# Spockuto/drand

Measured on AMD Instinct MI355X. Metric: beacons verified/s (batch chain verify), higher is better.
Workload: dtype u32 (381-bit Montgomery, 12x32-bit limbs); 1 GPU; configs[1]: 1000000-round chained beacon history per GPU, chain.VerifyBeacon per round; beacons_per_gpu=1000000, segment_len=64, parallelism=range-shard x1

## Files before the change

drand_amd/csrc/blsverify.cpp:

```cpp
#include <hip/hip_runtime.h>
#include <sys/random.h>

#include <algorithm>
#include <initializer_list>
#include <cerrno>
#include <cstdarg>
#include <cstdio>
#include <cstring>
#include <string>
#include <cstdlib>
#include <thread>
#include <vector>

#include "../../include/blsverify.h"
#include "../../include/blsverify_testing.h"
#include "kernels.h"
#include "engine_ctx.h"
#include "testops_list.h"

void release_workspace(blsv_ctx* c) {
  for (DBuf* d : {&c->H, &c->HQ, &c->S, &c->F, &c->FW, &c->LN, &c->h_inf, &c->s_inf, &c->cls}) d->release();
  c->cap = 0;
}

// ... 266 lines not shown
int blsv_test_lagrange(const uint32_t* idx, size_t t, uint32_t* out) {
  if (!idx || !out) return BLSV_EINVAL;
  for (size_t i = 0; i < t; i++)
    for (size_t j = 0; j < i; j++)
      if (idx[i] == idx[j]) return BLSV_EINVAL;
  host_lagrange(idx, t, out);
  return BLSV_OK;
}

struct PkSel {
  const uint32_t* tab;
  const uint8_t* inf;
  const uint32_t* idx;
};

static bool serial_stages() {
  static const bool on = [] {
    const char* e = getenv("BLSV_SERIAL_STAGES");
    return e && e[0] == '1';
  }();
  return on;
}

template <typename HashFn>
static int run_head(blsv_ctx* c, const uint8_t* d_sigs, size_t stride, size_t offset, size_t base, size_t cnt,
                    hipStream_t st, HashFn hash) {
  if (serial_stages()) {
    {
      StageTimer tm(c, ST_DECOMP, cnt, st);
      blsk::launch_decompress_g2(d_sigs, stride, offset, base, cnt, c->S.as<uint32_t>(), c->s_inf.as<uint8_t>(),
                                 c->cls.as<uint8_t>(), st);
    }
    StageTimer tm(c, ST_HASH, cnt, st);
    hash();
    return BLSV_OK;
  }
  HIPCHK(c, hipEventRecord(c->fork_ev, st));
  HIPCHK(c, hipStreamWaitEvent(c->side, c->fork_ev, 0));
  {
    StageTimer tm(c, ST_DECOMP, cnt, c->side);
    blsk::launch_decompress_g2(d_sigs, stride, offset, base, cnt, c->S.as<uint32_t>(), c->s_inf.as<uint8_t>(),
                               c->cls.as<uint8_t>(), c->side);
  }
  HIPCHK(c, hipEventRecord(c->join_ev, c->side));
  {
    StageTimer tm(c, ST_HASH, cnt, st);
    hash();
  }
  HIPCHK(c, hipStreamWaitEvent(st, c->join_ev, 0));
  return BLSV_OK;
}

static int run_tail(blsv_ctx* c, const uint8_t* d_sigs, size_t stride, size_t offset, size_t base, size_t cnt,
                    const PkSel& pk, uint64_t* d_bitmap, unsigned long long* d_first_bad, uint8_t* d_cls_out,
                    hipStream_t st, uint64_t label0 = 0) {
  (void)d_sigs;
  (void)stride;
  (void)offset;
  {
    StageTimer tm(c, ST_MILLER, cnt, st);
    blsk::launch_miller(pk.tab, pk.inf, pk.idx, c->H.as<uint32_t>(), c->h_inf.as<uint8_t>(), c->S.as<uint32_t>(),
                        c->s_inf.as<uint8_t>(), c->cls.as<uint8_t>(), cnt, c->F.as<uint32_t>(), c->LN.as<uint32_t>(),
                        std::min(cnt, kLineSub), c->FW.as<uint32_t>(), st);
  }
  {
    StageTimer tm(c, ST_FEXP, cnt, st);
    blsk::launch_final_exp(c->F.as<uint32_t>(), c->FW.as<uint32_t>(), cnt, c->cls.as<uint8_t>(), st,
                           c->LN.as<uint32_t>());
  }
  {
    StageTimer tm(c, ST_FINISH, cnt, st);
    blsk::launch_finish(c->cls.as<uint8_t>(), base, cnt, d_bitmap, d_first_bad, label0, st);
  }
  if (d_cls_out) HIPCHK(c, hipMemcpyAsync(d_cls_out + base, c->cls.p, cnt, hipMemcpyDeviceToDevice, st));
  HIPCHK(c, hipGetLastError());
  return BLSV_OK;
}

static void bitmap_words_to_bytes(const std::vector<uint64_t>& w, size_t n, uint8_t* out) {
  for (size_t i = 0; i < (n + 7) / 8; i++) {
    uint8_t b = (uint8_t)(w[i / 8] >> (8 * (i % 8)));
    if (i == (n + 7) / 8 - 1 && (n % 8)) b &= (uint8_t)((1u << (n % 8)) - 1);
    out[i] = b;
  }
}

// ... 33 lines not shown
    uint8_t* cls = reject_class;
    if (!cls) {
      own.resize(n);
      cls = own.data();
    }
    HIPCHK(c, download_sync(c, {{cls, c->cls.p, n}}));
    uint64_t fb = UINT64_MAX;
    for (size_t i = 0; i < n; i++) {
      if (cls[i] != BLSV_REJ_OK && fb == UINT64_MAX) fb = i;
      if (ok_bitmap) {
        if (i % 8 == 0) ok_bitmap[i / 8] = 0;
        ok_bitmap[i / 8] |= (uint8_t)((cls[i] == BLSV_REJ_OK) << (i % 8));
      }
    }
    if (first_bad_idx) *first_bad_idx = fb;
    return BLSV_OK;
  }
  HIPCHK(c, c->bitmap.ensure(words * 8 + 8));
  HIPCHK(c, c->first_bad.ensure(8));
  HIPCHK(c, hipMemsetAsync(c->first_bad.p, 0xff, 8, c->stream));
  if (reject_class) HIPCHK(c, c->misc.ensure(n + 64));
  for (size_t base = 0; base < n; base += c->cap) {
    const size_t cnt = std::min(c->cap, n - base);
    rc = run_head(c, d_sigs, stride, offset, base, cnt, c->stream, [&]() { hash(base, cnt); });
    if (rc) return rc;
    rc = run_tail(c, d_sigs, stride, offset, base, cnt, pk, c->bitmap.as<uint64_t>(),
                  c->first_bad.as<unsigned long long>(), reject_class ? c->misc.as<uint8_t>() : nullptr, c->stream);
    if (rc) return rc;
  }
  std::vector<uint64_t> w(words + 1, 0);
  uint64_t fb = UINT64_MAX;
  HIPCHK(c, download_sync(c, {{w.data(), c->bitmap.p, words * 8},
                              {&fb, c->first_bad.p, 8},
                              {reject_class, c->misc.p, reject_class ? n : 0}}));
  if (ok_bitmap) bitmap_words_to_bytes(w, n, ok_bitmap);
  if (first_bad_idx) *first_bad_idx = fb;
  return BLSV_OK;
}

static PkSel group_pk(blsv_ctx* c) { return {c->commits.as<uint32_t>(), c->commit_inf.as<uint8_t>(), nullptr}; }

static bool use_rlc(const blsv_ctx* c, size_t n) { return n > c->lat_max && n >= 2 * c->rlc.group; }

static int rlc_draw_seed(blsv_ctx* c, uint32_t (&w)[8]) {
  uint8_t s[32];
  if (c->rlc.seed_pinned) {
    memcpy(s, c->rlc.seed, 32);
// ... 15 lines not shown

static int rlc_sums(blsv_ctx* c, size_t base, size_t cnt, const uint32_t (&seed)[8], hipStream_t st) {
  rlc_state& r = c->rlc;
  const size_t ng = blsk::rlc_groups(cnt, r.group), cap = round64(ng);
  HIPCHK(c, r.part.ensure(2 * blsk::kRlcPartWords * blsk::rlc_lanes(cnt) * 4));
  HIPCHK(c, r.gH.ensure(cap * blsk::H_WORDS * 4));
  HIPCHK(c, r.gS.ensure(cap * blsk::S_WORDS * 4));
  HIPCHK(c, r.g_hinf.ensure(cap));
  HIPCHK(c, r.g_sinf.ensure(cap));
  HIPCHK(c, r.gcls.ensure(cap));
  StageTimer tm(c, ST_RLC, cnt, st);
  blsk::launch_rlc_sums(c->H.as<uint32_t>(), c->h_inf.as<uint8_t>(), c->S.as<uint32_t>(), c->s_inf.as<uint8_t>(),
                        c->cls.as<uint8_t>(), cnt, base, seed, r.group, r.part.as<uint32_t>(), r.gH.as<uint32_t>(),
                        r.g_hinf.as<uint8_t>(), r.gS.as<uint32_t>(), r.g_sinf.as<uint8_t>(), st);
  return BLSV_OK;
}

static void rlc_pairing_check(blsv_ctx* c, const uint32_t* H, const uint8_t* h_inf, const uint32_t* S,
                              const uint8_t* s_inf, uint8_t* cls, size_t cnt, hipStream_t st) {
  const PkSel pk = group_pk(c);
  {
    StageTimer tm(c, ST_MILLER, cnt, st);
    blsk::launch_miller(pk.tab, pk.inf, pk.idx, H, h_inf, S, s_inf, cls, cnt, c->F.as<uint32_t>(),
                        c->LN.as<uint32_t>(), std::min(cnt, kLineSub), c->FW.as<uint32_t>(), st);
  }
  StageTimer tm(c, ST_FEXP, cnt, st);
  blsk::launch_final_exp(c->F.as<uint32_t>(), c->FW.as<uint32_t>(), cnt, cls, st, c->LN.as<uint32_t>());
}

static int run_tail_rlc(blsv_ctx* c, size_t base, size_t cnt, const uint32_t (&seed)[8], uint64_t* d_bitmap,
                        unsigned long long* d_first_bad, uint8_t* d_cls_out, hipStream_t st, uint64_t label0 = 0) {
  rlc_state& r = c->rlc;
  const size_t G = r.group, ng = blsk::rlc_groups(cnt, G);
  int rc = rlc_sums(c, base, cnt, seed, st);
  if (rc) return rc;
  HIPCHK(c, hipMemsetAsync(r.gcls.p, 0, ng, st));
  rlc_pairing_check(c, r.gH.as<uint32_t>(), r.g_hinf.as<uint8_t>(), r.gS.as<uint32_t>(), r.g_sinf.as<uint8_t>(),
                    r.gcls.as<uint8_t>(), ng, st);
  HIPCHK(c, hipGetLastError());
  HIPCHK(c, r.host.ensure(kMaxChunk / kRlcGroupMin * 5 + 16));
  uint8_t* verdict = r.host.as<uint8_t>();
  HIPCHK(c, hipMemcpyAsync(verdict, r.gcls.p, ng, hipMemcpyDeviceToHost, st));
  HIPCHK(c, hipStreamSynchronize(st));
  uint32_t* fail_list = reinterpret_cast<uint32_t*>(verdict + ((ng + 7) & ~size_t(7)));
  size_t nf = 0;
  for (size_t g = 0; g < ng; g++)
    if (verdict[g] != BLSV_REJ_OK) fail_list[nf++] = (uint32_t)g;
// ... 25 lines not shown
    StageTimer tm(c, ST_FINISH, cnt, st);
    blsk::launch_finish(c->cls.as<uint8_t>(), base, cnt, d_bitmap, d_first_bad, label0, st);
  }
  if (d_cls_out) HIPCHK(c, hipMemcpyAsync(d_cls_out + base, c->cls.p, cnt, hipMemcpyDeviceToDevice, st));
  HIPCHK(c, hipGetLastError());
  return BLSV_OK;
}

template <typename HashFn>
static int verify_driver_rlc(blsv_ctx* c, size_t n, const uint8_t* d_sigs, HashFn hash, uint8_t* ok_bitmap,
                             uint64_t* first_bad_idx, uint8_t* reject_class) {
  const size_t words = (n + 63) / 64;
  int rc = ensure_workspace(c, n);
  if (rc) return rc;
  uint32_t seed[8];
  rc = rlc_draw_seed(c, seed);
  if (rc) return rc;
  HIPCHK(c, c->bitmap.ensure(words * 8 + 8));
  HIPCHK(c, c->first_bad.ensure(8));
  HIPCHK(c, hipMemsetAsync(c->first_bad.p, 0xff, 8, c->stream));
  if (reject_class) HIPCHK(c, c->misc.ensure(n + 64));
  for (size_t base = 0; base < n; base += c->cap) {
    const size_t cnt = std::min(c->cap, n - base);
    rc = run_head(c, d_sigs, 96, 0, base, cnt, c->stream, [&]() { hash(base, cnt); });
    if (rc) return rc;
    rc = run_tail_rlc(c, base, cnt, seed, c->bitmap.as<uint64_t>(), c->first_bad.as<unsigned long long>(),
                      reject_class ? c->misc.as<uint8_t>() : nullptr, c->stream);
    if (rc) return rc;
  }
  std::vector<uint64_t> w(words + 1, 0);
  uint64_t fb = UINT64_MAX;
  HIPCHK(c, download_sync(c, {{w.data(), c->bitmap.p, words * 8},
                              {&fb, c->first_bad.p, 8},
                              {reject_class, c->misc.p, reject_class ? n : 0}}));
  if (ok_bitmap) bitmap_words_to_bytes(w, n, ok_bitmap);
  if (first_bad_idx) *first_bad_idx = fb;
  return BLSV_OK;
}

static int decode_g1(blsv_ctx* c, const uint8_t* pk48, size_t cnt, DBuf& tab, DBuf& inf, std::vector<uint8_t>& cls) {
  HIPCHK(c, tab.ensure(cnt * blsk::G1_WORDS * 4));
  HIPCHK(c, inf.ensure(cnt));
  HIPCHK(c, c->g1_cls.ensure(cnt));
  HIPCHK(c, c->misc.ensure(cnt * 48));
  HIPCHK(c, hipMemcpyAsync(c->misc.p, pk48, cnt * 48, hipMemcpyHostToDevice, c->stream));
  blsk::launch_decompress_g1(c->misc.as<uint8_t>(), cnt, tab.as<uint32_t>(), inf.as<uint8_t>(),
                             c->g1_cls.as<uint8_t>(), c->stream);
// ... 38 lines not shown
  memcpy(h + o_idx, idx, n * 4);
  memcpy(h + o_sig, sigs96, n * 96);
  if (mbytes) memcpy(h + o_msg, msgs, mbytes);
  HIPCHK(c, c->arena.ensure(total));
  HIPCHK(c, c->misc.ensure(n + 64));
  HIPCHK(c, hipMemcpyAsync(c->arena.p, h, total, hipMemcpyHostToDevice, c->stream));
  uint8_t* d = c->arena.as<uint8_t>();
  const uint64_t* d_off = reinterpret_cast<const uint64_t*>(d);
  const uint32_t* d_len = reinterpret_cast<const uint32_t*>(d + o_len);
  const uint32_t* d_idx = reinterpret_cast<const uint32_t*>(d + o_idx);
  const uint8_t* d_sig = d + o_sig;
  const uint8_t* d_msg = d + o_msg;
  if (use_lat(c, n)) {
    blsk::launch_lat_messages(d_msg, d_off, d_len, d_sig, 96, 0, n, d_tab, d_tab_inf, d_idx, c->misc.as<uint8_t>(),
                              nullptr, nullptr, c->stream);
  } else {
    const size_t words = (n + 63) / 64;
    HIPCHK(c, c->bitmap.ensure(words * 8 + 8));
    HIPCHK(c, c->first_bad.ensure(8));
    HIPCHK(c, hipMemsetAsync(c->first_bad.p, 0xff, 8, c->stream));
    for (size_t base = 0; base < n; base += c->cap) {
      const size_t cnt = std::min(c->cap, n - base);
      const PkSel pk{d_tab, d_tab_inf, d_idx + base};
      rc = run_head(c, d_sig, 96, 0, base, cnt, c->stream, [&]() {
        blsk::launch_hash_messages(d_msg, d_off + base, d_len + base, cnt, c->H.as<uint32_t>(), c->h_inf.as<uint8_t>(),
                                   c->HQ.as<uint32_t>(), c->stream);
      });
      if (rc) return rc;
      rc = run_tail(c, d_sig, 96, 0, base, cnt, pk, c->bitmap.as<uint64_t>(), c->first_bad.as<unsigned long long>(),
                    c->misc.as<uint8_t>(), c->stream);
      if (rc) return rc;
    }
  }
  HIPCHK(c, hipGetLastError());
  HIPCHK(c, hipMemcpyAsync(h, c->misc.p, n, hipMemcpyDeviceToHost, c->stream));
  HIPCHK(c, hipStreamSynchronize(c->stream));
  memcpy(cls_out, h, n);
  return BLSV_OK;
}

extern "C" {

const char* blsv_version(void) { return "drand_amd blsverify 0.1 (gfx950)"; }

int blsv_device_count(void) {
  int n = 0;
  return hipGetDeviceCount(&n) == hipSuccess ? n : 0;
// ... 335 lines not shown
    HIPCHK(c, c->pp_inf.ensure(k));
    HIPCHK(c, c->sel.ensure(k * 4));
    ident.resize(k);
    for (size_t i = 0; i < k; i++) ident[i] = (uint32_t)i;
    HIPCHK(c, h2d(c, c->sel.p, ident.data(), k * 4));
    blsk::launch_pubpoly_eval(c->commits.as<uint32_t>(), c->commit_inf.as<uint8_t>(), (uint32_t)c->t,
                              c->idx.as<uint32_t>(), k, c->pp_tab.as<uint32_t>(), c->pp_inf.as<uint8_t>(), c->stream);
    pk = {c->pp_tab.as<uint32_t>(), c->pp_inf.as<uint8_t>(), c->sel.as<uint32_t>()};
  }
  HIPCHK(c, c->in_sigs.ensure(k * partial_len + 96));
  HIPCHK(c, h2d(c, c->in_sigs.p, partials, k * partial_len));
  if (use_lat(c, k)) {
    StageTimer tm(c, ST_LAT, k, c->stream);
    blsk::launch_lat_messages(c->in_msgs.as<uint8_t>(), c->in_off.as<uint64_t>(), c->in_len.as<uint32_t>(),
                              c->in_sigs.as<uint8_t>(), partial_len, 2, k, pk.tab, pk.inf, pk.idx, c->cls.as<uint8_t>(),
                              c->S.as<uint32_t>(), c->s_inf.as<uint8_t>(), c->stream);
    HIPCHK(c, hipGetLastError());
  } else {
    HIPCHK(c, c->bitmap.ensure(((k + 63) / 64) * 8 + 8));
    HIPCHK(c, c->first_bad.ensure(8));
    HIPCHK(c, hipMemsetAsync(c->first_bad.p, 0xff, 8, c->stream));
    blsk::launch_hash_messages(c->in_msgs.as<uint8_t>(), c->in_off.as<uint64_t>(), c->in_len.as<uint32_t>(), k,
                               c->H.as<uint32_t>(), c->h_inf.as<uint8_t>(), c->HQ.as<uint32_t>(), c->stream);
    rc = run_head(c, c->in_sigs.as<uint8_t>(), partial_len, 2, 0, k, c->stream, []() {});
    if (rc) return rc;
    rc = run_tail(c, c->in_sigs.as<uint8_t>(), partial_len, 2, 0, k, pk, c->bitmap.as<uint64_t>(),
                  c->first_bad.as<unsigned long long>(), nullptr, c->stream);
    if (rc) return rc;
  }
  HIPCHK(c, download_sync(c, {{cls.data(), c->cls.p, k}}));
  return BLSV_OK;
}

int blsv_verify_partials(blsv_ctx* c, const uint8_t* msg, size_t msg_len, const uint8_t* partials, size_t partial_len,
                         size_t k, uint8_t* ok, uint8_t* reject_class) {
  if (!c) return BLSV_EINVAL;
  if ((k && (!partials || !ok)) || (msg_len && !msg)) return fail(c, BLSV_EINVAL, "verify_partials: null arguments");
  (void)hipSetDevice(c->device);
  std::vector<uint8_t> cls;
  std::vector<uint32_t> index;
  int rc = partials_stage(c, msg, msg_len, partials, partial_len, k, cls, index);
  if (rc) return rc;
  for (size_t i = 0; i < k; i++) {
    ok[i] = cls[i] == BLSV_REJ_OK;
    if (reject_class) reject_class[i] = cls[i];
  }
  return BLSV_OK;
// ... 350 lines not shown
                            const uint8_t* d_seeds96, size_t seed0_len, const uint8_t* d_sigs96, size_t n,
                            uint64_t* d_bitmap, uint64_t* d_first_bad, uint8_t* d_reject_class, void* stream) {
  if (!c) return BLSV_EINVAL;
  if (!c->has_group) return fail(c, BLSV_ENOGROUP, "verify_chained_dev: no group key set");
  if (n && (!d_seeds96 || !d_sigs96 || !d_bitmap || !d_first_bad || (seed0_len != 32 && seed0_len != 96)))
    return fail(c, BLSV_EINVAL, "verify_chained_dev: bad arguments");
  if (seg_phase && (!seg_len || seg_phase >= seg_len))
    return fail(c, BLSV_EINVAL, "verify_chained_dev: seg_phase must be < seg_len");
  (void)hipSetDevice(c->device);
  hipStream_t st = stream ? (hipStream_t)stream : c->stream;
  HIPCHK(c, hipMemsetAsync(d_first_bad, 0xff, 8, st));
  int rc = ensure_workspace(c, n);
  if (rc) return rc;
  blsk::ChainedSrc src{d_sigs96, d_seeds96, first_round, seg_len ? seg_len : std::max<uint64_t>(n, 1),
                       (uint32_t)seed0_len, seg_phase};
  if (use_lat(c, n)) {
    const PkSel pk = group_pk(c);
    return run_lat(
        c, n, [&](uint8_t* cls) { blsk::launch_lat_chained(src, 0, n, pk.tab, pk.inf, cls, st); }, d_bitmap,
        (unsigned long long*)d_first_bad, d_reject_class, st, first_round);
  }
  for (size_t base = 0; base < n; base += c->cap) {
    const size_t cnt = std::min(c->cap, n - base);
    rc = run_head(c, d_sigs96, 96, 0, base, cnt, st, [&]() {
      blsk::launch_hash_chained(src, base, cnt, c->H.as<uint32_t>(), c->h_inf.as<uint8_t>(), c->HQ.as<uint32_t>(), st);
    });
    if (rc) return rc;
    rc = run_tail(c, d_sigs96, 96, 0, base, cnt, group_pk(c), d_bitmap, (unsigned long long*)d_first_bad,
                  d_reject_class, st, first_round);
    if (rc) return rc;
  }
  return BLSV_OK;
}

int blsv_generate_chained_dev(blsv_ctx* c, const uint8_t* sk32, uint64_t first_round, uint64_t seg_len,
                              const uint8_t* d_seeds96, size_t seed0_len, uint8_t* d_sigs96, size_t n, void* stream) {
  if (!c) return BLSV_EINVAL;
  if (!sk32 || (n && (!d_seeds96 || !d_sigs96)) || (seed0_len != 32 && seed0_len != 96))
    return fail(c, BLSV_EINVAL, "generate_chained_dev: bad arguments");
  (void)hipSetDevice(c->device);
  hipStream_t st = stream ? (hipStream_t)stream : c->stream;
  uint32_t sk[8];
  scalar_mod_r(sk32, sk);
  HIPCHK(c, c->sk.ensure(32));
  HIPCHK(c, hipMemcpyAsync(c->sk.p, sk, 32, hipMemcpyHostToDevice, st));
  blsk::ChainedSrc src{d_sigs96, d_seeds96, first_round, seg_len ? seg_len : std::max<uint64_t>(n, 1),
                       (uint32_t)seed0_len};
// ... 63 lines not shown
int blsv_verify_chained_rlc_dev(blsv_ctx* c, uint64_t first_round, uint64_t seg_len, uint64_t seg_phase,
                                const uint8_t* d_seeds96, size_t seed0_len, const uint8_t* d_sigs96, size_t n,
                                uint64_t* d_bitmap, uint64_t* d_first_bad, uint8_t* d_reject_class, void* stream) {
  if (!c) return BLSV_EINVAL;
  if (!use_rlc(c, n))
    return blsv_verify_chained_dev(c, first_round, seg_len, seg_phase, d_seeds96, seed0_len, d_sigs96, n, d_bitmap,
                                   d_first_bad, d_reject_class, stream);
  if (!c->has_group) return fail(c, BLSV_ENOGROUP, "verify_chained_rlc_dev: no group key set");
  if (!d_seeds96 || !d_sigs96 || !d_bitmap || !d_first_bad || (seed0_len != 32 && seed0_len != 96))
    return fail(c, BLSV_EINVAL, "verify_chained_rlc_dev: bad arguments");
  if (seg_phase && (!seg_len || seg_phase >= seg_len))
    return fail(c, BLSV_EINVAL, "verify_chained_rlc_dev: seg_phase must be < seg_len");
  (void)hipSetDevice(c->device);
  hipStream_t st = stream ? (hipStream_t)stream : c->stream;
  uint32_t seed[8];
  int rc = rlc_draw_seed(c, seed);
  if (rc) return rc;
  HIPCHK(c, hipMemsetAsync(d_first_bad, 0xff, 8, st));
  rc = ensure_workspace(c, n);
  if (rc) return rc;
  blsk::ChainedSrc src{d_sigs96, d_seeds96, first_round, seg_len ? seg_len : n, (uint32_t)seed0_len, seg_phase};
  for (size_t base = 0; base < n; base += c->cap) {
    const size_t cnt = std::min(c->cap, n - base);
    rc = run_head(c, d_sigs96, 96, 0, base, cnt, st, [&]() {
      blsk::launch_hash_chained(src, base, cnt, c->H.as<uint32_t>(), c->h_inf.as<uint8_t>(), c->HQ.as<uint32_t>(), st);
    });
    if (rc) return rc;
    rc = run_tail_rlc(c, base, cnt, seed, d_bitmap, (unsigned long long*)d_first_bad, d_reject_class, st, first_round);
    if (rc) return rc;
  }
  return BLSV_OK;
}

size_t blsv_set_rlc_group(blsv_ctx* c, size_t g) {
  if (!c) return 0;
  const size_t prev = c->rlc.group;
  size_t v = kRlcGroupMin;
  while (v * 2 <= g && v < kRlcGroupMax) v *= 2;
  c->rlc.group = v;
  return prev;
}

int blsv_rlc_stats(blsv_ctx* c, uint64_t* groups, uint64_t* groups_failed, uint64_t* items_exact) {
  if (!c) return BLSV_EINVAL;
  if (groups) *groups = c->rlc.groups;
  if (groups_failed) *groups_failed = c->rlc.groups_failed;
  if (items_exact) *items_exact = c->rlc.items_exact;
// ... 7 lines not shown
  return BLSV_OK;
}

int blsv_test_rlc_sums(blsv_ctx* c, uint64_t first_round, const uint8_t* prev0, size_t prev0_len,
                       const uint8_t* sigs96, size_t n, uint8_t* out_a96, uint8_t* out_b96) {
  if (!c) return BLSV_EINVAL;
  if (!n || !sigs96 || !prev0 || !out_a96 || !out_b96 || (prev0_len != 32 && prev0_len != 96))
    return fail(c, BLSV_EINVAL, "test_rlc_sums: bad arguments");
  (void)hipSetDevice(c->device);
  uint32_t seed[8];
  int rc = rlc_draw_seed(c, seed);
  if (rc) return rc;
  rc = ensure_workspace(c, n);
  if (rc) return rc;
  HIPCHK(c, c->in_sigs.ensure(n * 96 + 96));
  HIPCHK(c, c->seeds.ensure(96));
  HIPCHK(c, h2d(c, c->in_sigs.p, sigs96, n * 96));
  HIPCHK(c, h2d(c, c->seeds.p, prev0, prev0_len));
  blsk::ChainedSrc src{c->in_sigs.as<uint8_t>(), c->seeds.as<uint8_t>(), first_round, n, (uint32_t)prev0_len};
  rlc_state& r = c->rlc;
  size_t done = 0;
  for (size_t base = 0; base < n; base += c->cap) {
    const size_t cnt = std::min(c->cap, n - base), ng = blsk::rlc_groups(cnt, r.group);
    rc = run_head(c, c->in_sigs.as<uint8_t>(), 96, 0, base, cnt, c->stream, [&]() {
      blsk::launch_hash_chained(src, base, cnt, c->H.as<uint32_t>(), c->h_inf.as<uint8_t>(), c->HQ.as<uint32_t>(),
                                c->stream);
    });
    if (rc) return rc;
    rc = rlc_sums(c, base, cnt, seed, c->stream);
    if (rc) return rc;
    HIPCHK(c, r.out96.ensure(2 * ng * 96));
    uint8_t* d_out = r.out96.as<uint8_t>();
    blsk::launch_rlc_compress(r.gH.as<uint32_t>(), r.g_hinf.as<uint8_t>(), ng, d_out, c->stream);
    blsk::launch_rlc_compress(r.gS.as<uint32_t>(), r.g_sinf.as<uint8_t>(), ng, d_out + ng * 96, c->stream);
    HIPCHK(c, hipGetLastError());
    HIPCHK(c, hipMemcpyAsync(out_a96 + done * 96, d_out, ng * 96, hipMemcpyDeviceToHost, c->stream));
    HIPCHK(c, hipMemcpyAsync(out_b96 + done * 96, d_out + ng * 96, ng * 96, hipMemcpyDeviceToHost, c->stream));
    HIPCHK(c, hipStreamSynchronize(c->stream));
    c->io_up_off = 0;
    done += ng;
  }
  return (int)done;
}


static int tlock_prepare_sig(blsv_ctx* c, const uint8_t* sig96, hipStream_t st, uint8_t* sig_class) {
  tlock_state& t = c->tlock;
// ... 342 lines not shown
```

drand_amd/csrc/k_decomp.hip:

```cpp
#define BLS_FP2_KARA_INL 1
#include "kcommon.h"

namespace blsk {

#ifndef BLS_WPE_SUBGROUP
#define BLS_WPE_SUBGROUP 2
#endif

BLS_KERNEL(BLS_WPE_DECOMP) k_decompress_g2(const uint8_t* sigs, size_t stride, size_t offset, size_t base,
                                           size_t cnt, uint32_t* S, uint8_t* s_inf, uint8_t* cls) {
  size_t i = (size_t)blockIdx.x * TPB + threadIdx.x;
  if (i >= cnt) return;
  uint8_t buf[96];
  const uint8_t* p = sigs + (base + i) * stride + offset;
  for (int k = 0; k < 96; k++) buf[k] = p[k];
  g2a a;
  bool inf;
  uint8_t c = g2_decompress(buf, a, inf, false);
  if (c != REJ_OK) {
    a.x = fp2_zero();
    a.y = fp2_zero();
    inf = true;
  }
  st_fp2(S, cnt, i, 0, a.x);
// ... 63 lines not shown
  const bool in = i < cnt;
  const bool ok = in && cls[i] == REJ_OK;
  const bool bad = in && !ok;
  const unsigned long long okm = __ballot(ok);
  const unsigned long long badm = __ballot(bad);
  const int lane = threadIdx.x & 63;
  const size_t wave0 = i - lane;
  if (lane == 0 && wave0 < cnt) {
    bitmap[(base + wave0) >> 6] = okm;
    if (badm) atomicMin(first_bad, (unsigned long long)(label0 + base + wave0 + __builtin_ctzll(badm)));
  }
}

void launch_decompress_g2(const uint8_t* sigs, size_t stride, size_t offset, size_t base, size_t cnt, uint32_t* S,
                          uint8_t* s_inf, uint8_t* cls, hipStream_t st) {
  if (!cnt) return;
  hipLaunchKernelGGL(k_decompress_g2, dim3(grid_for(cnt)), dim3(TPB), 0, st, sigs, stride, offset, base, cnt, S,
                     s_inf, cls);
  hipLaunchKernelGGL(k_subgroup_g2, dim3(grid_for(cnt)), dim3(TPB), 0, st, S, s_inf, cls, cnt);
  hipLaunchKernelGGL(k_subgroup_g2_generic, dim3(grid_for(cnt)), dim3(TPB), 0, st, S, s_inf, cls, cnt,
                     g_generic_chains_all);
}

void launch_decompress_g2_only(const uint8_t* sigs, size_t stride, size_t offset, size_t cnt, uint32_t* S,
                               uint8_t* s_inf, uint8_t* cls, hipStream_t st) {
  if (!cnt) return;
  hipLaunchKernelGGL(k_decompress_g2, dim3(grid_for(cnt)), dim3(TPB), 0, st, sigs, stride, offset, size_t(0), cnt, S,
                     s_inf, cls);
}

void launch_finish(const uint8_t* cls, size_t base, size_t cnt, uint64_t* bitmap, unsigned long long* first_bad,
                   uint64_t label0, hipStream_t st) {
  if (!cnt) return;
  hipLaunchKernelGGL(k_finish, dim3((unsigned)((cnt + 255) / 256)), dim3(256), 0, st, cls, base, cnt, bitmap,
                     first_bad, label0);
}

}
```

drand_amd/csrc/k_miller.hip:

```cpp
#include "kcommon.h"
#include "testops.h"

namespace blsk {

DI int line_slot(int step, int k) { return (step * 2 + k) * 6; }
#ifndef BLS_LN_AUX
#define BLS_LN_AUX 2
#endif
#ifndef BLS_LN_AUX_ST
#define BLS_LN_AUX_ST BLS_LN_AUX
#endif
#ifndef BLS_LN_AUX_LD
#define BLS_LN_AUX_LD BLS_LN_AUX
#endif

static __shared__ uint32_t g_ml_T[72 * BLS_LANES];
struct g2proj_lds {
  uint32_t* base;
  DI fp2 get(int c) const {
    fp2 v;
#pragma unroll
    for (int w = 0; w < 12; w++) {
      v.c0.l[w] = base[(24 * c + w) * BLS_LANES];
      v.c1.l[w] = base[(24 * c + 12 + w) * BLS_LANES];
    }
    return v;
  }
  DI void set(int c, const fp2& v) const {
#pragma unroll
    for (int w = 0; w < 12; w++) {
      base[(24 * c + w) * BLS_LANES] = v.c0.l[w];
      base[(24 * c + 12 + w) * BLS_LANES] = v.c1.l[w];
    }
  }
};

BLS_KERNEL(BLS_WPE_LINES)
k_miller_lines(const uint32_t* pk_tab, const uint8_t* pk_inf, const uint32_t* pk_idx, const uint32_t* H,
               const uint8_t* h_inf, const uint32_t* S, const uint8_t* s_inf, const uint8_t* cls, size_t cnt,
               size_t base, size_t m, size_t sub, uint32_t* LN) {
  const int k = (int)(blockIdx.x & 1u);
  const size_t i = (size_t)(blockIdx.x >> 1) * TPB + threadIdx.x;
  if (i >= m) return;
  const size_t g = base + i;
  if (cls[g] != REJ_OK) return;
  const uint32_t kk = pk_idx ? pk_idx[g] : 0u;
  const bool act[2] = {!(pk_inf[kk] | h_inf[g]), !s_inf[g]};
  {
    const uint32_t* Qb = k == 0 ? H : S;
    auto load_q = [&]() {
      size_t j = g;
      asm volatile("" : "+v"(j));
      return g2a{ld_fp2(Qb, cnt, j, 0), ld_fp2(Qb, cnt, j, 2)};
    };
    auto emit = [&](int step, const line& l) {
      const int s = line_slot(step, k);
      const line o = act[k] ? l : line_one();
      st_fp2<BLS_LN_AUX_ST>(LN, sub, i, s + 0, o.a0);
      st_fp2<BLS_LN_AUX_ST>(LN, sub, i, s + 2, o.a1);
      st_fp2<BLS_LN_AUX_ST>(LN, sub, i, s + 4, o.a4);
    };
    auto pcoord = [&](int c) {
      size_t o = (size_t)kk * G1_WORDS + 12 * c;
// ... 6 lines not shown
    if (!act[k]) {
#pragma unroll 1
      for (int s = 0; s < MILLER_STEPS; s++) emit(s, line_one());
      return;
    }
    int step = 0;
    auto put = [&](int c, const fp2& v) { st_fp2<BLS_LN_AUX_ST>(LN, sub, i, line_slot(step, k) + 2 * c, v); };
    auto xp = [&]() { return pcoord(0); };
    auto yp = [&]() { return pcoord(1); };
    const g2proj_lds T{g_ml_T + threadIdx.x};
    {
      const g2a Q0 = load_q();
      T.set(0, Q0.x);
      T.set(1, Q0.y);
      T.set(2, fp2_one());
    }
#pragma unroll 1
    for (int b = 62; b >= 0; b--) {
      miller_dbl_step_ts(T, put, xp, yp);
      step++;
      if ((BLS_X_ABS >> b) & 1ull) {
        miller_add_step_ts(T, load_q, put, xp, yp);
        step++;
      }
    }
  }
}

static __shared__ uint32_t g_mf_L[120 * BLS_LANES];
DI void mf_put(int c, const fp2& v) {
  const unsigned l = threadIdx.x;
#pragma unroll
  for (int k = 0; k < 12; k++) {
    g_mf_L[(c * 24 + k) * BLS_LANES + l] = v.c0.l[k];
    g_mf_L[(c * 24 + 12 + k) * BLS_LANES + l] = v.c1.l[k];
  }
}
DI fp2 mf_get(int c) {
  unsigned l = threadIdx.x;
  asm volatile("" : "+v"(l));
  fp2 v;
#pragma unroll
  for (int k = 0; k < 12; k++) {
    v.c0.l[k] = g_mf_L[(c * 24 + k) * BLS_LANES + l];
    v.c1.l[k] = g_mf_L[(c * 24 + 12 + k) * BLS_LANES + l];
  }
// ... 151 lines not shown
  } else {
#pragma unroll
    for (int c = 0; c < 5; c++) mf_put(c, t_f2(x, 12 + 2 * c));
    t_put12(r, 0, fp12_mul_by_line_pair_lds(t_f12(x, 0)));
  }
#pragma unroll
  for (int k = 0; k < NOUT; k++)
#pragma unroll
    for (int w = 0; w < 12; w++) out[(i * NOUT + k) * 12 + w] = r[k].l[w];
}

bool launch_test_op_mf(int op, const uint32_t* in, size_t cnt, uint32_t* out, hipStream_t st) {
  if (op != TOP_fp6_mul_lb && op != TOP_fp12_mul_by_line_pair_lds) return false;
  if (!cnt) return true;
  if (op == TOP_fp6_mul_lb)
    hipLaunchKernelGGL((k_test_op_mf<TOP_fp6_mul_lb, 12, 6>), dim3(grid_for(cnt)), dim3(TPB), 0, st, in, cnt, out);
  else
    hipLaunchKernelGGL((k_test_op_mf<TOP_fp12_mul_by_line_pair_lds, 22, 12>), dim3(grid_for(cnt)), dim3(TPB), 0, st, in,
                       cnt, out);
  return true;
}

void launch_miller(const uint32_t* pk_tab, const uint8_t* pk_inf, const uint32_t* pk_idx, const uint32_t* H,
                   const uint8_t* h_inf, const uint32_t* S, const uint8_t* s_inf, const uint8_t* cls, size_t cnt,
                   uint32_t* F, uint32_t* LN, size_t sub, uint32_t* park, hipStream_t st) {
  if (!cnt) return;
  for (size_t b = 0; b < cnt; b += sub) {
    const size_t m = cnt - b < sub ? cnt - b : sub;
    hipLaunchKernelGGL(k_miller_lines, dim3(2 * grid_for(m)), dim3(TPB), 0, st, pk_tab, pk_inf, pk_idx, H, h_inf,
                       S, s_inf, cls, cnt, b, m, sub, LN);
    if (m <= kMillerTriMax) {
      hipLaunchKernelGGL(k_miller_f_tri, dim3((unsigned)((m + TRI_GROUPS - 1) / TRI_GROUPS)), dim3(TPB), 0, st, LN,
                         cls, cnt, b, m, sub, F, park);
    } else {
      hipLaunchKernelGGL(k_miller_f, dim3(grid_for(m)), dim3(TPB), 0, st, LN, cls, cnt, b, m, sub, F);
    }
  }
}

}
```

drand_amd/csrc/kernels.h:

```cpp
#pragma once
#include <hip/hip_runtime.h>
#include <stddef.h>
#include <stdint.h>

namespace blsk {

constexpr int H_WORDS = 48;
constexpr int S_WORDS = 48;
constexpr int F_WORDS = 144;
constexpr int G1_WORDS = 24;

struct ChainedSrc {
  const uint8_t* sigs;
  const uint8_t* seeds;
  uint64_t first_round;
  uint64_t seg_len;
  uint32_t seed0_len;
  uint64_t seg_phase;
};

constexpr int HQ_WORDS = 144;
void launch_hash_chained(const ChainedSrc& src, size_t base, size_t cnt, uint32_t* H, uint8_t* h_inf,
                         uint32_t* Q, hipStream_t st);
void launch_hash_unchained(const uint64_t* rounds, uint64_t first_round, size_t base, size_t cnt, uint32_t* H,
                           uint8_t* h_inf, uint32_t* Q, hipStream_t st);
void launch_hash_messages(const uint8_t* msgs, const uint64_t* off, const uint32_t* len, size_t cnt,
                          uint32_t* H, uint8_t* h_inf, uint32_t* Q, hipStream_t st);
void launch_decompress_g2(const uint8_t* sigs, size_t stride, size_t offset, size_t base, size_t cnt, uint32_t* S,
                          uint8_t* s_inf, uint8_t* cls, hipStream_t st);
constexpr int MILLER_LINE_WORDS = 68 * 2 * 6 * 12;
void launch_miller(const uint32_t* pk_tab, const uint8_t* pk_inf, const uint32_t* pk_idx, const uint32_t* H,
                   const uint8_t* h_inf, const uint32_t* S, const uint8_t* s_inf, const uint8_t* cls, size_t cnt,
                   uint32_t* F, uint32_t* LN, size_t sub, uint32_t* park, hipStream_t st);
constexpr size_t TRI_PARK_WORDS(size_t items) { return 48 * 64 * ((items + 20) / 21); }
constexpr size_t FEXP_PARK_WORDS(size_t items) { return TRI_PARK_WORDS(items); }
void launch_final_exp(uint32_t* F, uint32_t* W, size_t cnt, uint8_t* cls, hipStream_t st, uint32_t* park,
                      uint32_t* out = nullptr);
void launch_finish(const uint8_t* cls, size_t base, size_t cnt, uint64_t* bitmap, unsigned long long* first_bad,
                   uint64_t label0, hipStream_t st);

constexpr size_t kRlcLaneItems = 8;
constexpr size_t kRlcPartWords = 72;
constexpr size_t rlc_lanes(size_t cnt) { return (cnt + kRlcLaneItems - 1) / kRlcLaneItems; }
constexpr size_t rlc_groups(size_t cnt, size_t group) { return (cnt + group - 1) / group; }
void launch_rlc_sums(const uint32_t* H, const uint8_t* h_inf, const uint32_t* S, const uint8_t* s_inf,
                     const uint8_t* cls, size_t cnt, uint64_t index0, const uint32_t* seed_words, size_t group,
                     uint32_t* part, uint32_t* GH, uint8_t* g_hinf, uint32_t* GS, uint8_t* g_sinf, hipStream_t st);
void launch_rlc_gather(const uint32_t* fail, size_t group, size_t m, const uint32_t* H, const uint8_t* h_inf,
                       const uint32_t* S, const uint8_t* s_inf, const uint8_t* cls, size_t cnt, uint32_t* CH,
                       uint8_t* c_hinf, uint32_t* CS, uint8_t* c_sinf, uint8_t* ccls, hipStream_t st);
void launch_rlc_scatter(const uint32_t* fail, size_t group, size_t m, const uint8_t* ccls, uint8_t* cls, size_t cnt,
                        hipStream_t st);
void launch_rlc_compress(const uint32_t* GP, const uint8_t* g_inf, size_t ng, uint8_t* out96, hipStream_t st);

constexpr size_t kTlockTabWords = 68 * 3 * 24;
void launch_tlock_prepare(const uint32_t* S, const uint8_t* s_inf, const uint8_t* s_cls, uint32_t* tab, hipStream_t st);
void launch_tlock_f(const uint32_t* tab, const uint32_t* U, const uint8_t* u_inf, const uint8_t* cls,
                    const uint8_t* sig_inf, size_t cnt, uint32_t* F, hipStream_t st);
void launch_tlock_encode(const uint32_t* E, const uint8_t* cls, size_t cnt, uint8_t* out, hipStream_t st);

int lat_trace_read(uint64_t* out, int n, hipStream_t st);
int lat_trace_clear(hipStream_t st);
int lat_trace_enable(int on, hipStream_t st);
extern int g_generic_chains_all;
void launch_lat_chained(const ChainedSrc& src, size_t base, size_t cnt, const uint32_t* pk_tab, const uint8_t* pk_inf,
                        uint8_t* cls, hipStream_t st);
void launch_lat_unchained(const uint64_t* rounds, uint64_t first_round, const uint8_t* sigs, size_t base, size_t cnt,
                          const uint32_t* pk_tab, const uint8_t* pk_inf, uint8_t* cls, hipStream_t st);
void launch_lat_messages(const uint8_t* msgs, const uint64_t* off, const uint32_t* len, const uint8_t* sigs,
                         size_t stride, size_t offset, size_t cnt, const uint32_t* pk_tab, const uint8_t* pk_inf,
                         const uint32_t* pk_idx, uint8_t* cls, uint32_t* S, uint8_t* s_inf, hipStream_t st);

void launch_decompress_g1(const uint8_t* in, size_t cnt, uint32_t* tab, uint8_t* inf, uint8_t* cls, hipStream_t st);
void launch_pubpoly_eval(const uint32_t* commits, const uint8_t* commit_inf, uint32_t t, const uint32_t* idx,
                         size_t cnt, uint32_t* out_tab, uint8_t* out_inf, hipStream_t st);
void launch_lat_decode(const uint8_t* sigs, size_t stride, size_t offset, size_t cnt, uint32_t* S, uint8_t* s_inf,
                       uint8_t* cls, hipStream_t st);
void launch_decompress_g2_only(const uint8_t* sigs, size_t stride, size_t offset, size_t cnt, uint32_t* S,
                               uint8_t* s_inf, uint8_t* cls, hipStream_t st);
void launch_lat_recover(const uint32_t* S, size_t n_s, const uint8_t* s_inf, const uint32_t* sel,
                        const uint32_t* lambdas, uint32_t t, uint32_t* scratch, uint8_t* out96, hipStream_t st,
                        uint32_t* saff = nullptr);
constexpr size_t kLatHoutWords = 448, kLatSaffWords = 192;
void launch_lat_hash_key(const uint8_t* msgs, const uint64_t* off, const uint32_t* len, const uint32_t* pk_tab,
                         const uint8_t* pk_inf, uint32_t* hout, hipStream_t st);
void launch_lat_verify_pre(const uint32_t* hout, const uint32_t* saff, uint8_t* cls, hipStream_t st);
void launch_sign(const uint32_t* sk_words, int32_t index, const uint32_t* H, const uint8_t* h_inf, size_t cnt,
                 uint8_t* out, size_t out_stride, hipStream_t st);
void launch_gen_chained(const uint32_t* sk_words, const ChainedSrc& src, size_t n, uint8_t* sigs_out, hipStream_t st);

bool launch_test_op(int op, const uint32_t* in, size_t cnt, uint32_t* out, uint32_t* park, hipStream_t st);
bool launch_test_op_mf(int op, const uint32_t* in, size_t cnt, uint32_t* out, hipStream_t st);
void launch_test_fp_mul(const uint32_t* a, const uint32_t* b, size_t cnt, uint32_t* out, hipStream_t st);
void launch_test_pairing(const uint32_t* p_tab, const uint32_t* q_aff, size_t cnt, uint32_t* out_f, hipStream_t st);
void launch_test_unpack_g2(const uint32_t* H, size_t cnt, uint32_t* out, hipStream_t st);
void launch_test_pack_fp12(const uint32_t* f, size_t cnt, uint32_t* F, hipStream_t st);
void launch_test_unpack_fp12(const uint32_t* F, size_t cnt, uint32_t* out, hipStream_t st);
void launch_test_final_exp_ref(const uint32_t* F, size_t cnt, uint32_t* out, hipStream_t st);

}
```

drand_amd/csrc/pairing.h:

```cpp
#pragma once
#include "curve.h"

namespace bls {

struct g2proj {
  fp2 x, y, z;
};

DI fp2 fp2_mul_3b(const fp2& c) {
  fp2 x4 = fp2_dbl(fp2_dbl(fp2_mul_xi(c)));
  return fp2_add(fp2_dbl(x4), x4);
}

template <bool INL = false>
DI void miller_dbl_step(g2proj& t, fp2& l00, fp2& l01, fp2& l11, const fp& xp, const fp& yp) {
  auto mul = [](const fp2& a, const fp2& b) { return INL ? fp2_mul_inl(a, b) : fp2_mul(a, b); };
  auto sqr = [](const fp2& a) { return INL ? fp2_sqr_inl(a) : fp2_sqr(a); };
  fp2 A = fp2_half(mul(t.x, t.y));
  fp2 B = sqr(t.y);
  fp2 C = sqr(t.z);
  fp2 E = fp2_mul_3b(C);
  fp2 F = fp2_mul3(E);
  fp2 G = fp2_half(fp2_add(B, F));
  fp2 H = fp2_sub(sqr(fp2_add_lazy(t.y, t.z)), fp2_add(B, C));
// ... 62 lines not shown
  }
  put(1, fp2_neg(fp2_mul_fp_inl(theta, xp())));
  BLS_SCHED_FENCE();
  put(2, fp2_mul_fp_inl(delta, yp()));
  BLS_SCHED_FENCE();
  const fp2 C = fp2_sqr_inl(theta);
  BLS_SCHED_FENCE();
  const fp2 D = fp2_sqr_inl(delta);
  BLS_SCHED_FENCE();
  const fp2 E = fp2_mul_inl(D, delta);
  BLS_SCHED_FENCE();
  const fp2 F = fp2_mul_inl(t.get(2), C);
  BLS_SCHED_FENCE();
  const fp2 G = fp2_mul_inl(t.get(0), D);
  BLS_SCHED_FENCE();
  const fp2 H = fp2_sub(fp2_add(E, F), fp2_dbl(G));
  t.set(0, fp2_mul_inl(delta, H));
  BLS_SCHED_FENCE();
  t.set(1, fp2_sub(fp2_mul_inl(theta, fp2_sub(G, H)), fp2_mul_inl(t.get(1), E)));
  BLS_SCHED_FENCE();
  t.set(2, fp2_mul_inl(t.get(2), E));
}

template <typename Put, typename XP, typename YP>
DI void miller_dbl_step_inl(g2proj& t, Put put, XP xp, YP yp) {
  miller_dbl_step_ts(g2proj_reg{t}, put, xp, yp);
}
template <typename Put, typename Q, typename XP, typename YP>
DI void miller_add_step_inl(g2proj& t, Q qload, Put put, XP xp, YP yp) {
  miller_add_step_ts(g2proj_reg{t}, qload, put, xp, yp);
}

DI void miller_add_step(g2proj& t, const g2a& q, fp2& l00, fp2& l01, fp2& l11, const fp& xp, const fp& yp) {
  fp2 theta = fp2_sub(t.y, fp2_mul(q.y, t.z));
  fp2 delta = fp2_sub(t.x, fp2_mul(q.x, t.z));
  l00 = fp2_sub(fp2_mul(theta, q.x), fp2_mul(delta, q.y));
  l01 = fp2_neg(fp2_mul_fp(theta, xp));
  l11 = fp2_mul_fp(delta, yp);
  fp2 C = fp2_sqr(theta);
  fp2 D = fp2_sqr(delta);
  fp2 E = fp2_mul(D, delta);
  fp2 F = fp2_mul(t.z, C);
  fp2 G = fp2_mul(t.x, D);
  fp2 H = fp2_sub(fp2_add(E, F), fp2_dbl(G));
  t.x = fp2_mul(delta, H);
  t.y = fp2_sub(fp2_mul(theta, fp2_sub(G, H)), fp2_mul(t.y, E));
// ... 169 lines not shown
```

Baseline: 2.320 million beacons/s.

## Fuse G2 subgroup check into Miller loop using final T accumulator

The separate subgroup check that ran during signature decompression is dropped in the non-RLC paths. Instead, after the Miller loop's doubling/addition chain over |x|, the signature-side thread compares the accumulated point T against psi(Q) (with negation) to decide subgroup membership. This reuses the scalar multiplication already done by the Miller loop, removing a costly independent scalar multiplication per signature. The cost is a few extra Fp2 multiplications and a cls write in the line kernel, plus reliance on the psi-based membership criterion being correct.

```diff
diff --git a/drand_amd/csrc/blsverify.cpp b/drand_amd/csrc/blsverify.cpp
--- a/drand_amd/csrc/blsverify.cpp
+++ b/drand_amd/csrc/blsverify.cpp
@@ -312,14 +312,23 @@
   return on;
 }
 
+static void head_decompress(blsv_ctx* c, const uint8_t* d_sigs, size_t stride, size_t offset, size_t base, size_t cnt,
+                            bool fused_subgroup, hipStream_t st) {
+  if (fused_subgroup && !blsk::g_generic_chains_all)
+    blsk::launch_decompress_g2_only(d_sigs, stride, offset, base, cnt, c->S.as<uint32_t>(), c->s_inf.as<uint8_t>(),
+                                    c->cls.as<uint8_t>(), st);
+  else
+    blsk::launch_decompress_g2(d_sigs, stride, offset, base, cnt, c->S.as<uint32_t>(), c->s_inf.as<uint8_t>(),
+                               c->cls.as<uint8_t>(), st);
+}
+
 template <typename HashFn>
 static int run_head(blsv_ctx* c, const uint8_t* d_sigs, size_t stride, size_t offset, size_t base, size_t cnt,
-                    hipStream_t st, HashFn hash) {
+                    bool fused_subgroup, hipStream_t st, HashFn hash) {
   if (serial_stages()) {
     {
       StageTimer tm(c, ST_DECOMP, cnt, st);
-      blsk::launch_decompress_g2(d_sigs, stride, offset, base, cnt, c->S.as<uint32_t>(), c->s_inf.as<uint8_t>(),
-                                 c->cls.as<uint8_t>(), st);
+      head_decompress(c, d_sigs, stride, offset, base, cnt, fused_subgroup, st);
     }
     StageTimer tm(c, ST_HASH, cnt, st);
     hash();
@@ -329,8 +338,7 @@
   HIPCHK(c, hipStreamWaitEvent(c->side, c->fork_ev, 0));
   {
     StageTimer tm(c, ST_DECOMP, cnt, c->side);
-    blsk::launch_decompress_g2(d_sigs, stride, offset, base, cnt, c->S.as<uint32_t>(), c->s_inf.as<uint8_t>(),
-                               c->cls.as<uint8_t>(), c->side);
+    head_decompress(c, d_sigs, stride, offset, base, cnt, fused_subgroup, c->side);
   }
   HIPCHK(c, hipEventRecord(c->join_ev, c->side));
   {
@@ -351,7 +359,7 @@
     StageTimer tm(c, ST_MILLER, cnt, st);
     blsk::launch_miller(pk.tab, pk.inf, pk.idx, c->H.as<uint32_t>(), c->h_inf.as<uint8_t>(), c->S.as<uint32_t>(),
                         c->s_inf.as<uint8_t>(), c->cls.as<uint8_t>(), cnt, c->F.as<uint32_t>(), c->LN.as<uint32_t>(),
-                        std::min(cnt, kLineSub), c->FW.as<uint32_t>(), st);
+                        std::min(cnt, kLineSub), c->FW.as<uint32_t>(), true, st);
   }
   {
     StageTimer tm(c, ST_FEXP, cnt, st);
@@ -431,7 +439,7 @@
   if (reject_class) HIPCHK(c, c->misc.ensure(n + 64));
   for (size_t base = 0; base < n; base += c->cap) {
     const size_t cnt = std::min(c->cap, n - base);
-    rc = run_head(c, d_sigs, stride, offset, base, cnt, c->stream, [&]() { hash(base, cnt); });
+    rc = run_head(c, d_sigs, stride, offset, base, cnt, true, c->stream, [&]() { hash(base, cnt); });
     if (rc) return rc;
     rc = run_tail(c, d_sigs, stride, offset, base, cnt, pk, c->bitmap.as<uint64_t>(),
                   c->first_bad.as<unsigned long long>(), reject_class ? c->misc.as<uint8_t>() : nullptr, c->stream);
@@ -493,7 +501,7 @@
   {
     StageTimer tm(c, ST_MILLER, cnt, st);
     blsk::launch_miller(pk.tab, pk.inf, pk.idx, H, h_inf, S, s_inf, cls, cnt, c->F.as<uint32_t>(),
-                        c->LN.as<uint32_t>(), std::min(cnt, kLineSub), c->FW.as<uint32_t>(), st);
+                        c->LN.as<uint32_t>(), std::min(cnt, kLineSub), c->FW.as<uint32_t>(), false, st);
   }
   StageTimer tm(c, ST_FEXP, cnt, st);
   blsk::launch_final_exp(c->F.as<uint32_t>(), c->FW.as<uint32_t>(), cnt, cls, st, c->LN.as<uint32_t>());
@@ -565,7 +573,7 @@
   if (reject_class) HIPCHK(c, c->misc.ensure(n + 64));
   for (size_t base = 0; base < n; base += c->cap) {
     const size_t cnt = std::min(c->cap, n - base);
-    rc = run_head(c, d_sigs, 96, 0, base, cnt, c->stream, [&]() { hash(base, cnt); });
+    rc = run_head(c, d_sigs, 96, 0, base, cnt, false, c->stream, [&]() { hash(base, cnt); });
     if (rc) return rc;
     rc = run_tail_rlc(c, base, cnt, seed, c->bitmap.as<uint64_t>(), c->first_bad.as<unsigned long long>(),
                       reject_class ? c->misc.as<uint8_t>() : nullptr, c->stream);
@@ -650,7 +658,7 @@
     for (size_t base = 0; base < n; base += c->cap) {
       const size_t cnt = std::min(c->cap, n - base);
       const PkSel pk{d_tab, d_tab_inf, d_idx + base};
-      rc = run_head(c, d_sig, 96, 0, base, cnt, c->stream, [&]() {
+      rc = run_head(c, d_sig, 96, 0, base, cnt, true, c->stream, [&]() {
         blsk::launch_hash_messages(d_msg, d_off + base, d_len + base, cnt, c->H.as<uint32_t>(), c->h_inf.as<uint8_t>(),
                                    c->HQ.as<uint32_t>(), c->stream);
       });
@@ -1032,7 +1040,7 @@
     HIPCHK(c, hipMemsetAsync(c->first_bad.p, 0xff, 8, c->stream));
     blsk::launch_hash_messages(c->in_msgs.as<uint8_t>(), c->in_off.as<uint64_t>(), c->in_len.as<uint32_t>(), k,
                                c->H.as<uint32_t>(), c->h_inf.as<uint8_t>(), c->HQ.as<uint32_t>(), c->stream);
-    rc = run_head(c, c->in_sigs.as<uint8_t>(), partial_len, 2, 0, k, c->stream, []() {});
+    rc = run_head(c, c->in_sigs.as<uint8_t>(), partial_len, 2, 0, k, true, c->stream, []() {});
     if (rc) return rc;
     rc = run_tail(c, c->in_sigs.as<uint8_t>(), partial_len, 2, 0, k, pk, c->bitmap.as<uint64_t>(),
                   c->first_bad.as<unsigned long long>(), nullptr, c->stream);
@@ -1429,7 +1437,7 @@
   }
   for (size_t base = 0; base < n; base += c->cap) {
     const size_t cnt = std::min(c->cap, n - base);
-    rc = run_head(c, d_sigs96, 96, 0, base, cnt, st, [&]() {
+    rc = run_head(c, d_sigs96, 96, 0, base, cnt, true, st, [&]() {
       blsk::launch_hash_chained(src, base, cnt, c->H.as<uint32_t>(), c->h_inf.as<uint8_t>(), c->HQ.as<uint32_t>(), st);
     });
     if (rc) return rc;
@@ -1539,7 +1547,7 @@
   blsk::ChainedSrc src{d_sigs96, d_seeds96, first_round, seg_len ? seg_len : n, (uint32_t)seed0_len, seg_phase};
   for (size_t base = 0; base < n; base += c->cap) {
     const size_t cnt = std::min(c->cap, n - base);
-    rc = run_head(c, d_sigs96, 96, 0, base, cnt, st, [&]() {
+    rc = run_head(c, d_sigs96, 96, 0, base, cnt, false, st, [&]() {
       blsk::launch_hash_chained(src, base, cnt, c->H.as<uint32_t>(), c->h_inf.as<uint8_t>(), c->HQ.as<uint32_t>(), st);
     });
     if (rc) return rc;
@@ -1593,7 +1601,7 @@
   size_t done = 0;
   for (size_t base = 0; base < n; base += c->cap) {
     const size_t cnt = std::min(c->cap, n - base), ng = blsk::rlc_groups(cnt, r.group);
-    rc = run_head(c, c->in_sigs.as<uint8_t>(), 96, 0, base, cnt, c->stream, [&]() {
+    rc = run_head(c, c->in_sigs.as<uint8_t>(), 96, 0, base, cnt, false, c->stream, [&]() {
       blsk::launch_hash_chained(src, base, cnt, c->H.as<uint32_t>(), c->h_inf.as<uint8_t>(), c->HQ.as<uint32_t>(),
                                 c->stream);
     });
diff --git a/drand_amd/csrc/k_decomp.hip b/drand_amd/csrc/k_decomp.hip
--- a/drand_amd/csrc/k_decomp.hip
+++ b/drand_amd/csrc/k_decomp.hip
@@ -109,10 +109,10 @@
                      g_generic_chains_all);
 }
 
-void launch_decompress_g2_only(const uint8_t* sigs, size_t stride, size_t offset, size_t cnt, uint32_t* S,
-                               uint8_t* s_inf, uint8_t* cls, hipStream_t st) {
+void launch_decompress_g2_only(const uint8_t* sigs, size_t stride, size_t offset, size_t base, size_t cnt,
+                               uint32_t* S, uint8_t* s_inf, uint8_t* cls, hipStream_t st) {
   if (!cnt) return;
-  hipLaunchKernelGGL(k_decompress_g2, dim3(grid_for(cnt)), dim3(TPB), 0, st, sigs, stride, offset, size_t(0), cnt, S,
+  hipLaunchKernelGGL(k_decompress_g2, dim3(grid_for(cnt)), dim3(TPB), 0, st, sigs, stride, offset, base, cnt, S,
                      s_inf, cls);
 }
 
diff --git a/drand_amd/csrc/k_miller.hip b/drand_amd/csrc/k_miller.hip
--- a/drand_amd/csrc/k_miller.hip
+++ b/drand_amd/csrc/k_miller.hip
@@ -1,3 +1,5 @@
+#include <type_traits>
+
 #include "kcommon.h"
 #include "testops.h"
 
@@ -35,10 +37,12 @@
   }
 };
 
+template <bool CHECK>
 BLS_KERNEL(BLS_WPE_LINES)
 k_miller_lines(const uint32_t* pk_tab, const uint8_t* pk_inf, const uint32_t* pk_idx, const uint32_t* H,
-               const uint8_t* h_inf, const uint32_t* S, const uint8_t* s_inf, const uint8_t* cls, size_t cnt,
-               size_t base, size_t m, size_t sub, uint32_t* LN) {
+               const uint8_t* h_inf, const uint32_t* S, const uint8_t* s_inf,
+               std::conditional_t<CHECK, uint8_t*, const uint8_t*> cls, size_t cnt, size_t base, size_t m, size_t sub,
+               uint32_t* LN) {
   const int k = (int)(blockIdx.x & 1u);
   const size_t i = (size_t)(blockIdx.x >> 1) * TPB + threadIdx.x;
   if (i >= m) return;
@@ -91,6 +95,13 @@
       if ((BLS_X_ABS >> b) & 1ull) {
         miller_add_step_ts(T, load_q, put, xp, yp);
         step++;
+      }
+    }
+    if constexpr (CHECK) {
+      if (k == 1 && !miller_t_in_subgroup(T, load_q)) {
+        size_t j = g;
+        asm volatile("" : "+v"(j));
+        cls[j] = REJ_NOT_IN_SUBGROUP;
       }
     }
   }
@@ -288,13 +299,17 @@
 }
 
 void launch_miller(const uint32_t* pk_tab, const uint8_t* pk_inf, const uint32_t* pk_idx, const uint32_t* H,
-                   const uint8_t* h_inf, const uint32_t* S, const uint8_t* s_inf, const uint8_t* cls, size_t cnt,
-                   uint32_t* F, uint32_t* LN, size_t sub, uint32_t* park, hipStream_t st) {
+                   const uint8_t* h_inf, const uint32_t* S, const uint8_t* s_inf, uint8_t* cls, size_t cnt,
+                   uint32_t* F, uint32_t* LN, size_t sub, uint32_t* park, bool check_subgroup, hipStream_t st) {
   if (!cnt) return;
   for (size_t b = 0; b < cnt; b += sub) {
     const size_t m = cnt - b < sub ? cnt - b : sub;
-    hipLaunchKernelGGL(k_miller_lines, dim3(2 * grid_for(m)), dim3(TPB), 0, st, pk_tab, pk_inf, pk_idx, H, h_inf,
-                       S, s_inf, cls, cnt, b, m, sub, LN);
+    if (check_subgroup)
+      hipLaunchKernelGGL(k_miller_lines<true>, dim3(2 * grid_for(m)), dim3(TPB), 0, st, pk_tab, pk_inf, pk_idx, H,
+                         h_inf, S, s_inf, cls, cnt, b, m, sub, LN);
+    else
+      hipLaunchKernelGGL(k_miller_lines<false>, dim3(2 * grid_for(m)), dim3(TPB), 0, st, pk_tab, pk_inf, pk_idx, H,
+                         h_inf, S, s_inf, (const uint8_t*)cls, cnt, b, m, sub, LN);
     if (m <= kMillerTriMax) {
       hipLaunchKernelGGL(k_miller_f_tri, dim3((unsigned)((m + TRI_GROUPS - 1) / TRI_GROUPS)), dim3(TPB), 0, st, LN,
                          cls, cnt, b, m, sub, F, park);
diff --git a/drand_amd/csrc/kernels.h b/drand_amd/csrc/kernels.h
--- a/drand_amd/csrc/kernels.h
+++ b/drand_amd/csrc/kernels.h
@@ -30,8 +30,8 @@
                           uint8_t* s_inf, uint8_t* cls, hipStream_t st);
 constexpr int MILLER_LINE_WORDS = 68 * 2 * 6 * 12;
 void launch_miller(const uint32_t* pk_tab, const uint8_t* pk_inf, const uint32_t* pk_idx, const uint32_t* H,
-                   const uint8_t* h_inf, const uint32_t* S, const uint8_t* s_inf, const uint8_t* cls, size_t cnt,
-                   uint32_t* F, uint32_t* LN, size_t sub, uint32_t* park, hipStream_t st);
+                   const uint8_t* h_inf, const uint32_t* S, const uint8_t* s_inf, uint8_t* cls, size_t cnt,
+                   uint32_t* F, uint32_t* LN, size_t sub, uint32_t* park, bool check_subgroup, hipStream_t st);
 constexpr size_t TRI_PARK_WORDS(size_t items) { return 48 * 64 * ((items + 20) / 21); }
 constexpr size_t FEXP_PARK_WORDS(size_t items) { return TRI_PARK_WORDS(items); }
 void launch_final_exp(uint32_t* F, uint32_t* W, size_t cnt, uint8_t* cls, hipStream_t st, uint32_t* park,
@@ -76,8 +76,8 @@
                          size_t cnt, uint32_t* out_tab, uint8_t* out_inf, hipStream_t st);
 void launch_lat_decode(const uint8_t* sigs, size_t stride, size_t offset, size_t cnt, uint32_t* S, uint8_t* s_inf,
                        uint8_t* cls, hipStream_t st);
-void launch_decompress_g2_only(const uint8_t* sigs, size_t stride, size_t offset, size_t cnt, uint32_t* S,
-                               uint8_t* s_inf, uint8_t* cls, hipStream_t st);
+void launch_decompress_g2_only(const uint8_t* sigs, size_t stride, size_t offset, size_t base, size_t cnt,
+                               uint32_t* S, uint8_t* s_inf, uint8_t* cls, hipStream_t st);
 void launch_lat_recover(const uint32_t* S, size_t n_s, const uint8_t* s_inf, const uint32_t* sel,
                         const uint32_t* lambdas, uint32_t t, uint32_t* scratch, uint8_t* out96, hipStream_t st,
                         uint32_t* saff = nullptr);
diff --git a/drand_amd/csrc/pairing.h b/drand_amd/csrc/pairing.h
--- a/drand_amd/csrc/pairing.h
+++ b/drand_amd/csrc/pairing.h
@@ -108,6 +108,23 @@
   t.set(2, fp2_mul_inl(t.get(2), E));
 }
 
+template <typename TS, typename Q>
+DI bool miller_t_in_subgroup(const TS& t, Q qload) {
+  bool ok = !fp2_is_zero(t.get(2));
+  {
+    const fp2 px = fp2_mul_inl(fp2_conj(qload().x), fp2_load_const(PSI_KX));
+    BLS_SCHED_FENCE();
+    ok &= fp2_eq(t.get(0), fp2_mul_inl(px, t.get(2)));
+  }
+  BLS_SCHED_FENCE();
+  {
+    const fp2 py = fp2_mul_inl(fp2_conj(qload().y), fp2_load_const(PSI_KY));
+    BLS_SCHED_FENCE();
+    ok &= fp2_eq(fp2_neg(t.get(1)), fp2_mul_inl(py, t.get(2)));
+  }
+  return ok;
+}
+
 template <typename Put, typename XP, typename YP>
 DI void miller_dbl_step_inl(g2proj& t, Put put, XP xp, YP yp) {
   miller_dbl_step_ts(g2proj_reg{t}, put, xp, yp);
```

Result: faster. 2.410 million beacons/s (median of 6 runs) (+3.9%).
